# carlosmwh1985/BspAtom

Measured on AMD Instinct MI355X. Metric: l-channel eigensolves/sec at N_bsp=4096 fp64, higher is better.
Workload: dtype f64; 1 GPU; Hydrogen Coulomb l=0..127, N_bsp=4096, k=9, KIND_GRID=0 rb=800 (BASELINE configs[3]); `value` = weak scaling: 128 l-channels per GPU, 128 in total; channels_total=128, eigenvector_owner_rank=0, collective_calls=0, launched_by=python

## Files before the change

### bspatom_amd/csrc/common.h

```cpp
#pragma once
#include <hip/hip_runtime.h>
#include <cstdint>
#include <cstdio>
#include <cstdlib>

#define BSP_OK 0
#define BSP_ERR_HIP (-1)
#define BSP_ERR_ARG (-2)
#define BSP_ERR_BSPLVB (-3)
#define BSP_ERR_NOGPU (-4)
#define BSP_ERR_UNSUPPORTED (-5)

#define BSP_HIP(x)                                                                          \
    do {                                                                                    \
        hipError_t e_ = (x);                                                                \
        if (e_ != hipSuccess) {                                                             \
            fprintf(stderr, "bspatom: HIP error '%s' at %s:%d\n", hipGetErrorString(e_),    \
                    __FILE__, __LINE__);                                                    \
            return BSP_ERR_HIP;                                                             \
        }                                                                                   \
    } while (0)

typedef double double4_t __attribute__((ext_vector_type(4)));

// ... 90 lines not shown
                    int part, hipStream_t st);
int symm_lower_f64(int m, int batch, const double *A22, long ld, long bsA, const double *W, long ldw, long bsW,
                   double *Y, long ldy, long bsY, hipStream_t st);

int launch_point_table(int nkp, int k, int ka, int nfun, const double *d_rt, const double *d_aind,
                       const double *d_xg, const double *d_wg, const double *d_vpot, double *d_ptab,
                       int *d_left, int *d_status, hipStream_t st);
int launch_assemble_bands(int nfun, int k, int ka, int nkp, int kind_pot, const double *d_bl, int l0,
                          int nl, const double *d_ptab, const int *d_left, double *d_SB, double *d_HB,
                          hipStream_t st);
int launch_dipole_bands(int nfun, int k, int ka, int nkp, const double *d_ptab, const int *d_left, double *d_RB,
                        hipStream_t st);
int launch_band_cholesky(int n, int k, const double *d_SB, double *d_UB, double *d_rdiag, int *d_info,
                         hipStream_t st);
int launch_band_cholesky_range(int n, int k, int jstart, int jstop, const double *d_SB, double *d_UB, double *d_rdiag, int *d_info,
                               hipStream_t st);
int launch_band_cholesky_pair(int n, int k, int jstop, const double *d_SB, double *d_UB, double *d_rdiag, int *d_info, hipStream_t st);
int launch_standard_form(int n, int npad, int k, int nl, const double *d_HB, const double *d_UB,
                         const double *d_rdiag, double *d_Y, double *d_C, hipStream_t st, int full = 0);
struct CrawfordWork {
    double *SBf, *UBf, *rdiagf;
    double *Qel, *LiB;
    double *D, *E, *G;
    int *info;
};
bool crawford_supported(int n, int k);
size_t crawford_work_bytes(int n, int k, int nl);
void crawford_carve(void *base, int n, int k, int nl, CrawfordWork *w);
constexpr int CW_CHUNKS = 4;
int crawford_prepare(int n, int k, const double *d_SB, const CrawfordWork &w, hipStream_t st, hipEvent_t *evc = nullptr);
int crawford_run(int n, int npad, int k, int nl, const double *d_SB, const double *d_HB, const CrawfordWork &w, double *d_AB,
                 hipStream_t st, bool s_prepared = false, hipEvent_t *evc = nullptr, hipStream_t aux0 = nullptr);
long tsqr_scr_doubles(int npad);
long tsqr_cntr_ints(int npad);
int tsqr_panel(int npad, int r0, int c0, int batch, double *d_A, double *buf, double *W, double *scr, int *cntr, hipStream_t st);
struct Sy2sbWork {
    double *tsqr_scr;
    int *tsqr_cntr;
    double *buf2;
    double *tau2;
    double *buf;
    double *W;
    double *G;
    double *T;
    double *Kmat;
    double *tau;
// ... 127 lines not shown
```

### bspatom_amd/csrc/crawford.hip

```cpp
#include "common.h"
#include <cstdio>
#include <mutex>

namespace bsp {
namespace {

constexpr int CB = 8;
constexpr int CBB = CB * CB;

template <int CTRL>
__device__ __forceinline__ double cw_dpp(double x)
{
    union { double d; int i[2]; } u, r;
    u.d = x;
    r.i[0] = __builtin_amdgcn_update_dpp(0, u.i[0], CTRL, 0xf, 0xf, true);
    r.i[1] = __builtin_amdgcn_update_dpp(0, u.i[1], CTRL, 0xf, 0xf, true);
    return r.d;
}
__device__ __forceinline__ double cw_rowsum(double x)
{
    x += cw_dpp<0x128>(x);
    x += cw_dpp<0x124>(x);
    x += cw_dpp<0x122>(x);
    x += cw_dpp<0x121>(x);
    return x;
}
__device__ __forceinline__ double cw_bperm(double x, int srclane)
{
    union { double d; int i[2]; } u, r;
    u.d = x;
    r.i[0] = __builtin_amdgcn_ds_bpermute(srclane << 2, u.i[0]);
// ... 30 lines not shown
    if (I > 0) {
        const double w0 = cw_rowsum(x0 * u);
        x0 = fma(-t * w0, u, x0);
    }
    if (I > 4) {
        const double w1 = cw_rowsum(x1 * u);
        x1 = fma(-t * w1, u, x1);
    }
    if (g == GI) xr = (c < LEN) ? 0.0 : ((c == LEN) ? beta : xr);
#pragma unroll
    for (int r = 0; r < 4; ++r) {
        const double wq = cw_rowsum(q[r] * u);
        q[r] = fma(-t * wq, u, q[r]);
    }
}

__device__ __forceinline__ double4_t cw_mfma(double a, double b, double4_t acc)
{
    return __builtin_amdgcn_mfma_f64_16x16x4f64(a, b, acc, 0, 0, 0);
}

template <bool ONEDIV>
__global__ __launch_bounds__(256) void crawford_item_kernel(int N, int t, int jlo, int nch, int jel, int nlh, int qstride, int nlead,
                                                           const double *__restrict__ Qel, double *Dall, double *Eall, double *Gall)
{
    if ((int)blockIdx.y >= nlh) {
        if (jlo + nch > nlead) nch = nlead > jlo ? nlead - jlo : 0;
        if (jel >= nlead) jel = 0;
    }
    const int lane = threadIdx.x & 63;
    const int idx = blockIdx.x * 4 + __builtin_amdgcn_readfirstlane(threadIdx.x >> 6);
    const int g = lane >> 4, c = lane & 15, c8 = c & 7;
    const bool left = c < CB;
    bool elim;
    int j, p;
    if (idx < nch) { elim = false; j = jlo + idx; p = j - 2 - (t - 2 * j); }
    else if (idx == nch && jel > 0) { elim = true; j = jel; p = j - 1; }
    else return;
    const size_t chn = (size_t)blockIdx.y * N * CBB;
    double *D = Dall + chn, *E = Eall + chn, *G = Gall + chn;
    double *D0 = D + (size_t)p * CBB, *D1 = D0 + CBB, *E0 = E + (size_t)p * CBB;

    double w[4], sd[2];
#pragma unroll
    for (int r = 0; r < 2; ++r) {
        const int R = 4 * r + g;
        const int hi = R > c8 ? R : c8, lo = R > c8 ? c8 : R;
        w[r] = *(left ? D0 + hi * CB + lo : E0 + c8 * CB + R);
        w[r + 2] = *(left ? E0 + R * CB + c8 : D1 + hi * CB + lo);
    }
    const bool side = p >= 1;
    {
        const double *Em = E + (size_t)(side ? p - 1 : 0) * CBB;
#pragma unroll
        for (int r = 0; r < 2; ++r) {
            const double v = Em[(4 * r + g) * CB + c8];
            sd[r] = (side && left) ? v : 0.0;
        }
    }
    double q[4], x0 = 0.0, x1 = 0.0, xt[2] = {0.0, 0.0};
    const bool has_x = elim && (j + 1 <= N - 1);
    if (!elim) {
        const double *src = left ? G + (size_t)p * CBB + c8 : E + (size_t)(p + 1) * CBB + c8;
        x0 = src[g * CB];
        x1 = src[(4 + g) * CB];
#pragma unroll
        for (int r = 0; r < 4; ++r) q[r] = (4 * r + g == c) ? 1.0 : 0.0;
        rq_step<7, ONEDIV>(x0, x1, q, g, c);
        rq_step<6, ONEDIV>(x0, x1, q, g, c);
        rq_step<5, ONEDIV>(x0, x1, q, g, c);
        rq_step<4, ONEDIV>(x0, x1, q, g, c);
        rq_step<3, ONEDIV>(x0, x1, q, g, c);
// ... 4 lines not shown
        const double *Qj = Qel + ((int)blockIdx.y >= nlh ? qstride : 0) + (size_t)j * 256;
#pragma unroll
        for (int r = 0; r < 4; ++r) q[r] = Qj[(4 * r + g) * 16 + c];
        const double *Ej = E + (size_t)(has_x ? j : 0) * CBB;
#pragma unroll
        for (int r = 0; r < 2; ++r) {
            const double v = Ej[c8 * CB + 4 * r + g];
            xt[r] = (has_x && left) ? v : 0.0;
        }
    }

    double4_t P = {0.0, 0.0, 0.0, 0.0}, Wn = {0.0, 0.0, 0.0, 0.0};
#pragma unroll
    for (int r = 0; r < 4; ++r) P = cw_mfma(w[r], q[r], P);
#pragma unroll
    for (int r = 0; r < 4; ++r) Wn = cw_mfma(q[r], P[r], Wn);
    double4_t O = {0.0, 0.0, 0.0, 0.0};
    O = cw_mfma(q[0], sd[0], O);
    O = cw_mfma(q[1], sd[1], O);

    if (left) {
#pragma unroll
        for (int r = 0; r < 2; ++r) {
            D0[(4 * r + g) * CB + c8] = Wn[r];
            E0[(4 * r + g) * CB + c8] = Wn[r + 2];
        }
    } else {
#pragma unroll
        for (int r = 0; r < 2; ++r) D1[(4 * r + g) * CB + c8] = Wn[r + 2];
    }
    if (side && left) {
        double *Em = E + (size_t)(p - 1) * CBB, *Gm = G + (size_t)(p - 1) * CBB;
#pragma unroll
        for (int r = 0; r < 2; ++r) {
            if (!elim) Em[(4 * r + g) * CB + c8] = O[r];
            Gm[(4 * r + g) * CB + c8] = O[r + 2];
        }
    }
    if (!elim) {
        if (!left) {
            double *E1 = E + (size_t)(p + 1) * CBB;
            E1[g * CB + c8] = x0;
            E1[(4 + g) * CB + c8] = x1;
        }
    } else if (has_x) {
        double4_t T = {0.0, 0.0, 0.0, 0.0};
        T = cw_mfma(q[2], xt[0], T);
        T = cw_mfma(q[3], xt[1], T);
        if (left) {
            double *Ej = E + (size_t)j * CBB;
#pragma unroll
            for (int r = 0; r < 2; ++r) Ej[c8 * CB + 4 * r + g] = T[r + 2];
// ... 155 lines not shown
        cw_baxpy<I, 0, 8>(x, u, tw);
        cw_baxpy<I, 8, I + 1>(x, u, tw);
    }
    {
        double ws[4] = {0.0, 0.0, 0.0, 0.0};
        cw_bdot<I, 0, 8>(ws, u, q);
        cw_bdot<I, 8, I + 1>(ws, u, q);
        const double w = (ws[0] + ws[1]) + (ws[2] + ws[3]);
        const double tw = -t * w;
        cw_baxpy<I, 0, 8>(q, u, tw);
        if constexpr (ONEDIV) {
            cw_baxpy<I, 8, I + 1>(q, u, tw);
        } else {
            if constexpr (I > 0) cw_baxpy_last<I, 8, I>(q, u, tw, -t, w);
            else q[LEN] = fma(-t, w, q[LEN]);
        }
    }
}

template <bool ONEDIV, bool BCAST>
__device__ __forceinline__ void cw_quad(const int N, const int t, const int jlo, int nch, int jel, const int ipw, const int nlh,
                                        const int qstride, const int nlead, const int chan, const int idx0, const int lane,
                                        double *Qsw, double *Bcw, double *Wsw, const double *__restrict__ Qel, double *Dall, double *Eall,
                                        double *Gall, unsigned long long *diag)
{
    unsigned long long ts0 = 0, tsa = 0, tsb = 0, tsc = 0, tsd = 0, tse = 0;
    if (diag) ts0 = __builtin_amdgcn_s_memtime();
    if (chan >= nlh) {
        if (jlo + nch > nlead) nch = nlead > jlo ? nlead - jlo : 0;
        if (jel >= nlead) jel = 0;
    }
    const int items = nch + (jel > 0 ? 1 : 0);
    if (idx0 >= items) return;
    const size_t chn = (size_t)chan * N * CBB;
    double *D = Dall + chn, *E = Eall + chn, *G = Gall + chn;

#pragma unroll
    for (int s = 0; s < 4; ++s) {
        const int idx = idx0 + s;
        const int kd = s >= ipw ? 0 : (idx < nch ? 1 : ((idx == nch && jel > 0) ? 2 : 0));
        if (kd != 0) {
            const int jx = kd == 1 ? jlo + idx : jel, p = kd == 2 ? jel - 1 : jx - 2 - (t - 2 * jx);
            const double *srcD = D + (size_t)p * CBB + 2 * lane;
            const double *srcE = E + (size_t)((lane < 32 || p < 1) ? p : p - 1) * CBB + 2 * (lane & 31);
            const unsigned ldsD = (unsigned)(size_t)(__attribute__((address_space(3))) void *)(Wsw + s * 4 * CBB);
            asm volatile("s_mov_b32 m0, %2\n\ts_nop 0\n\tglobal_load_lds_dwordx4 %0, off\n\t"
                         "s_mov_b32 m0, %3\n\ts_nop 0\n\tglobal_load_lds_dwordx4 %1, off"
                         :: "v"(srcD), "v"(srcE), "s"(ldsD), "s"(ldsD + 2 * CBB * 8) : "memory", "m0");
        }
    }

    double wv[4][4], sdv[4][2];
    auto read_ws = [&]() {
        const int g = lane >> 4, c8 = lane & 7;
        const bool left = (lane & 15) < CB;
#pragma unroll
        for (int s = 0; s < 4; ++s) {
            const double *W0 = Wsw + s * 4 * CBB, *W1 = W0 + CBB, *WE = W0 + 2 * CBB, *WM = W0 + 3 * CBB;
#pragma unroll
            for (int r = 0; r < 2; ++r) {
                const int R = 4 * r + g;
                const int hi = R > c8 ? R : c8, lo = R > c8 ? c8 : R;
                wv[s][r] = *(left ? W0 + hi * CB + lo : WE + c8 * CB + R);
                wv[s][r + 2] = *(left ? WE + R * CB + c8 : W1 + hi * CB + lo);
                sdv[s][r] = WM[(4 * r + g) * CB + c8];
            }
        }
    };

    if (idx0 < nch) {
        const int it = lane >> 4, r = lane & 15;
        const int idx = idx0 + it;
        const bool live = idx < nch && it < ipw && r < CB;
        const int j = jlo + (idx < nch ? idx : 0), p = j - 2 - (t - 2 * j);
        double x[16], q[16];
        {
            const double *gp = G + (size_t)p * CBB + (r & 7) * CB, *ep = E + (size_t)(p + 1) * CBB + (r & 7) * CB;
#pragma unroll
            for (int c = 0; c < CB; c += 2) {
                const double2 a = *reinterpret_cast<const double2 *>(gp + c), b = *reinterpret_cast<const double2 *>(ep + c);
                x[c] = live ? a.x : 0.0; x[c + 1] = live ? a.y : 0.0;
                x[CB + c] = live ? b.x : 0.0; x[CB + c + 1] = live ? b.y : 0.0;
            }
        }
#pragma unroll
        for (int c = 0; c < 16; ++c) q[c] = (c == r) ? 1.0 : 0.0;
        if (diag) { asm volatile("s_waitcnt vmcnt(0)" ::: "memory"); tsa = __builtin_amdgcn_s_memtime(); }
        if constexpr (BCAST) {
// ... 21 lines not shown
            double *ep = E + (size_t)(p + 1) * CBB + r * CB;
#pragma unroll
            for (int c = 0; c < CB; c += 2) *reinterpret_cast<double2 *>(ep + c) = make_double2(x[CB + c], x[CB + c + 1]);
        }
        if constexpr (BCAST) {
            asm volatile("s_waitcnt vmcnt(4)" ::: "memory");
            read_ws();
            asm volatile("" ::: "memory");
        }
        double *qs = Qsw + it * (16 * QLD) + r * QLD;
#pragma unroll
        for (int c = 0; c < 16; c += 2) *reinterpret_cast<double2 *>(qs + c) = make_double2(q[c], q[c + 1]);
    } else if constexpr (BCAST) {
        asm volatile("s_waitcnt vmcnt(0)" ::: "memory");
        read_ws();
    }
    if constexpr (BCAST) asm volatile("s_waitcnt lgkmcnt(0)" ::: "memory");
    else if (idx0 < nch) asm volatile("s_waitcnt vmcnt(4) lgkmcnt(0)" ::: "memory");
    else asm volatile("s_waitcnt vmcnt(0) lgkmcnt(0)" ::: "memory");
    if (diag) tsc = __builtin_amdgcn_s_memtime();
    int idx0b = idx0;
    size_t chnb = chn;
    asm volatile("" : "+s"(idx0b), "+s"(chnb));
    D = Dall + chnb; E = Eall + chnb; G = Gall + chnb;

    const int g = lane >> 4, c = lane & 15, c8 = c & 7;
    const bool left = c < CB;
    int kind[4], jj[4], pp[4];
    double qe[4], xt[2] = {0.0, 0.0};
    if constexpr (!BCAST) read_ws();
#pragma unroll
    for (int s = 0; s < 4; ++s) {
        const int idx = idx0b + s;
        kind[s] = s >= ipw ? 0 : (idx < nch ? 1 : ((idx == nch && jel > 0) ? 2 : 0));
        jj[s] = kind[s] == 1 ? jlo + idx : (kind[s] == 2 ? jel : jlo + idx0b);
        pp[s] = kind[s] == 2 ? jel - 1 : jj[s] - 2 - (t - 2 * jj[s]);
        if (kind[s] == 0) { jj[s] = jj[0]; pp[s] = pp[0]; }
#pragma unroll
        for (int r = 0; r < 2; ++r) sdv[s][r] = (pp[s] >= 1 && left) ? sdv[s][r] : 0.0;
    }
    int se = -1;
#pragma unroll
    for (int s = 0; s < 4; ++s) if (kind[s] == 2) se = s;
    const bool has_x = se >= 0 && (jel + 1 <= N - 1);
    if (se >= 0) {
        const double *Qj = Qel + ((int)chan >= nlh ? qstride : 0) + (size_t)jel * 256;
#pragma unroll
        for (int r = 0; r < 4; ++r) qe[r] = Qj[(4 * r + g) * 16 + c];
        const double *Ej = E + (size_t)(has_x ? jel : 0) * CBB;
#pragma unroll
        for (int r = 0; r < 2; ++r) {
            const double v = Ej[c8 * CB + 4 * r + g];
            xt[r] = (has_x && left) ? v : 0.0;
        }
    }
    if (diag) { asm volatile("s_waitcnt vmcnt(0)" ::: "memory"); tsd = __builtin_amdgcn_s_memtime(); }
#pragma unroll
    for (int s = 0; s < 4; ++s) {
        if (kind[s] == 0) break;
        const bool elim = kind[s] == 2;
        const int p = pp[s];
        double *D0 = D + (size_t)p * CBB, *D1 = D0 + CBB, *E0 = E + (size_t)p * CBB;
        double q[4];
        if (!elim) {
            const double *qs = Qsw + s * (16 * QLD);
#pragma unroll
            for (int r = 0; r < 4; ++r) q[r] = qs[(4 * r + g) * QLD + c];
        } else {
#pragma unroll
            for (int r = 0; r < 4; ++r) q[r] = qe[r];
        }
        double4_t P = {0.0, 0.0, 0.0, 0.0}, Wn = {0.0, 0.0, 0.0, 0.0};
#pragma unroll
        for (int r = 0; r < 4; ++r) P = cw_mfma(wv[s][r], q[r], P);
#pragma unroll
        for (int r = 0; r < 4; ++r) Wn = cw_mfma(q[r], P[r], Wn);
        double4_t O = {0.0, 0.0, 0.0, 0.0};
        O = cw_mfma(q[0], sdv[s][0], O);
        O = cw_mfma(q[1], sdv[s][1], O);
        if (left) {
#pragma unroll
            for (int r = 0; r < 2; ++r) {
                D0[(4 * r + g) * CB + c8] = Wn[r];
                E0[(4 * r + g) * CB + c8] = Wn[r + 2];
            }
        } else {
#pragma unroll
            for (int r = 0; r < 2; ++r) D1[(4 * r + g) * CB + c8] = Wn[r + 2];
        }
        if (p >= 1 && left) {
            double *Em = E + (size_t)(p - 1) * CBB, *Gm = G + (size_t)(p - 1) * CBB;
#pragma unroll
            for (int r = 0; r < 2; ++r) {
                if (!elim) Em[(4 * r + g) * CB + c8] = O[r];
                Gm[(4 * r + g) * CB + c8] = O[r + 2];
            }
        }
        if (elim && has_x) {
            double4_t T = {0.0, 0.0, 0.0, 0.0};
            T = cw_mfma(q[2], xt[0], T);
            T = cw_mfma(q[3], xt[1], T);
            if (left) {
                double *Ej = E + (size_t)jel * CBB;
#pragma unroll
                for (int r = 0; r < 2; ++r) Ej[c8 * CB + 4 * r + g] = T[r + 2];
            }
        }
    }
    if (diag) {
        tse = __builtin_amdgcn_s_memtime();
        asm volatile("s_waitcnt vmcnt(0)" ::: "memory");
        const unsigned long long tsf = __builtin_amdgcn_s_memtime();
        if (lane == 0) {
            const bool a = tsa != 0;
            atomicAdd(diag + 0, a ? tsa - ts0 : 0ull);
            atomicAdd(diag + 1, a ? tsb - tsa : 0ull);
            atomicAdd(diag + 2, a ? tsc - tsb : tsc - ts0);
            atomicAdd(diag + 3, tsd - tsc);
            atomicAdd(diag + 4, tse - tsd);
            atomicAdd(diag + 5, tsf - tse);
            atomicAdd(diag + 6, tsf - ts0);
            atomicAdd(diag + 7, 1ull);
        }
    }
}

template <bool ONEDIV, int NW, bool BCAST>
__global__ __launch_bounds__(64 * NW, (BCAST ? 16 : 8) / NW) void crawford_item4_kernel(int N, int t, int jlo, int nch, int jel, int ipw, int nlh, int qstride,
                                                            int nlead, const double *__restrict__ Qel, double *Dall, double *Eall, double *Gall,
                                                            unsigned long long *diag)
{
    __builtin_amdgcn_s_setprio(3);
    if (diag && (((blockIdx.x & 7) | (blockIdx.y & 7)) != 0)) diag = nullptr;
    __shared__ __attribute__((aligned(16))) double Qs[NW][4][16 * QLD];
    __shared__ __attribute__((aligned(16))) double Bc[BCAST ? 1 : NW][BCAST ? 1 : 4][BCAST ? 2 : 16];
    __shared__ __attribute__((aligned(16))) double Wsep[BCAST ? 1 : NW][BCAST ? 1 : 4][BCAST ? 2 : 4 * CBB];
    static_assert(16 * QLD >= 4 * CBB, "a slot of Q holds a slot of phase B's operands");
    double *Wsw = BCAST ? &Qs[0][0][0] : &Wsep[0][0][0];
    const int lane = threadIdx.x & 63;
    const int wave = __builtin_amdgcn_readfirstlane(threadIdx.x >> 6);
    cw_quad<ONEDIV, BCAST>(N, t, jlo, nch, jel, ipw, nlh, qstride, nlead, (int)blockIdx.y, (blockIdx.x * NW + wave) * ipw, lane,
                           &Qs[wave][0][0], BCAST ? nullptr : &Bc[wave][0][0], Wsw + wave * (BCAST ? 4 * 16 * QLD : 4 * 4 * CBB), Qel, Dall,
                           Eall, Gall, diag);
}

__global__ void crawford_flip_kernel(int n, int k, const double *__restrict__ SB, double *__restrict__ SBf)
{
    const int idx = blockIdx.x * blockDim.x + threadIdx.x;
    if (idx >= n * k) return;
    const int d = idx / n, i = idx % n;
    SBf[idx] = (i + d < n) ? SB[(size_t)d * n + (n - 1 - i - d)] : 0.0;
    SBf[(size_t)n * k + idx] = SB[idx];
}

__global__ __launch_bounds__(64) void crawford_setup_kernel(int n, int k, int fstride, int jfirst, const double *__restrict__ UB0,
                                                           double *__restrict__ LiB0, double *__restrict__ Qel0)
{
    __shared__ double Ld[CB][CB + 1], M[CB][CB + 1], Li[CB][CB + 1];
    const int j = jfirst + blockIdx.x, t = threadIdx.x, r = t >> 3, c = t & 7, b = k - 1;
    const double *UBf = UB0 + (size_t)blockIdx.y * k * n;
    double *LiB = LiB0 + (size_t)blockIdx.y * fstride * CBB, *Qel = Qel0 + (size_t)blockIdx.y * fstride * 256;
    const int i = CB * j + r;
    {
        const int ic = CB * j + c, d = r - c;
        double v = 0.0;
        if (i >= n) v = (r == c) ? 1.0 : 0.0;
// ... 12 lines not shown
        for (int rr = 0; rr < CB; ++rr) {
            double s = (rr == t) ? 1.0 : 0.0;
#pragma unroll
            for (int kk = 0; kk < CB; ++kk)
                if (kk < rr && kk >= t) s -= Ld[rr][kk] * x[kk];
            x[rr] = (rr >= t) ? s / Ld[rr][rr] : 0.0;
        }
#pragma unroll
        for (int rr = 0; rr < CB; ++rr) Li[rr][t] = x[rr];
    }
    __syncthreads();
    double kv = 0.0;
#pragma unroll
    for (int kk = 0; kk < CB; ++kk) kv += Li[r][kk] * M[kk][c];
    LiB[(size_t)j * CBB + t] = Li[r][c];
    double *Q = Qel + (size_t)j * 256;
    Q[r * 16 + c] = (r == c) ? 1.0 : 0.0;
    Q[c * 16 + CB + r] = -kv;
    Q[(CB + r) * 16 + c] = 0.0;
    Q[(CB + c) * 16 + CB + r] = Li[r][c];
}

__global__ __launch_bounds__(64) void crawford_init_kernel(int n, int k, int N, int nlh, int listride, const double *__restrict__ HBall,
                                                          const double *__restrict__ LiB, double *Dall, double *Eall)
{
    __shared__ double Ds[CB][CB + 1], Es[CB][CB + 1], Ls[CB][CB + 1], Ts[CB][CB + 1];
    const int p = blockIdx.x, t = threadIdx.x, r = t >> 3, c = t & 7, b = k - 1;
    const bool fwd = (int)blockIdx.y >= nlh;
    const double *HB = HBall + (size_t)(fwd ? blockIdx.y - nlh : blockIdx.y) * k * n;
    auto Hf = [&](int i, int i2) -> double {
        const int hi = i > i2 ? i : i2, lo = i > i2 ? i2 : i, d = hi - lo;
        return (hi < n && d <= b) ? HB[(size_t)d * n + (fwd ? lo : n - 1 - hi)] : 0.0;
    };
    double dv = Hf(CB * p + r, CB * p + c), ev = Hf(CB * (p + 1) + r, CB * p + c);
    if (p == 0) {
        Ds[r][c] = dv; Es[r][c] = ev; Ls[r][c] = LiB[(fwd ? listride : 0) + t];
        __syncthreads();
        double s = 0.0, e2 = 0.0;
#pragma unroll
        for (int kk = 0; kk < CB; ++kk) { s += Ls[r][kk] * Ds[kk][c]; e2 += Es[r][kk] * Ls[c][kk]; }
        Ts[r][c] = s;
        __syncthreads();
        s = 0.0;
#pragma unroll
        for (int kk = 0; kk < CB; ++kk) s += Ts[r][kk] * Ls[c][kk];
        dv = s; ev = e2;
    }
    const size_t o = ((size_t)blockIdx.y * N + p) * CBB + t;
    Dall[o] = dv;
    Eall[o] = ev;
}

__global__ __launch_bounds__(64) void crawford_cut_setup_kernel(int n, int k, int N, int Nh, int Nl, const double *__restrict__ SBf,
                                                               const double *__restrict__ LiB, double *__restrict__ Qel, int *info)
{
    __shared__ double A[CB][CB + 1], Lf[CB][CB + 1], T[CB][CB + 1], Gm[CB][CB + 1], Li[CB][CB + 1];
    const int t = threadIdx.x, r = t >> 3, c = t & 7, b = k - 1;
    const double *L0 = LiB + (size_t)(Nh - 1) * CBB, *L1 = LiB + (size_t)N * CBB + (size_t)(Nl - 1) * CBB;
    {
        const int d = CB + r - c;
        A[r][c] = (d <= b) ? SBf[(size_t)d * n + CB * (Nh - 1) + c] : 0.0;
        Lf[r][c] = L1[(CB - 1 - r) * CB + (CB - 1 - c)];
        Li[r][c] = 0.0;
    }
    __syncthreads();
    double v = 0.0;
#pragma unroll
    for (int q = 0; q < CB; ++q) v += Lf[r][q] * A[q][c];
    T[r][c] = v;
    __syncthreads();
    v = 0.0;
#pragma unroll
    for (int q = 0; q < CB; ++q) v += T[r][q] * L0[c * CB + q];
// ... 28 lines not shown
            for (int kk = 0; kk < CB; ++kk)
                if (kk < rr && kk >= t) sacc -= A[rr][kk] * x[kk];
            x[rr] = (rr >= t) ? sacc / A[rr][rr] : 0.0;
        }
#pragma unroll
        for (int rr = 0; rr < CB; ++rr) Li[rr][t] = x[rr];
    }
    __syncthreads();
    double kv = 0.0;
#pragma unroll
    for (int kk = 0; kk < CB; ++kk) kv += Li[r][kk] * Gm[kk][c];
    double *Q = Qel + (size_t)Nh * 256;
    Q[r * 16 + c] = (r == c) ? 1.0 : 0.0;
    Q[c * 16 + CB + r] = -kv;
    Q[(CB + r) * 16 + c] = 0.0;
    Q[(CB + c) * 16 + CB + r] = Li[r][c];
}

__global__ __launch_bounds__(64) void crawford_cut_prep_kernel(int N, int Nh, int Nl, int nl, int Nfull, const double *__restrict__ LiB,
                                                              double *Dall, double *Eall)
{
    __shared__ double X[CB][CB + 1], Lf[CB][CB + 1];
    const int t = threadIdx.x, r = t >> 3, c = t & 7;
    const size_t c0 = (size_t)blockIdx.x * N * CBB, c1 = (size_t)(nl + blockIdx.x) * N * CBB;
    const double *L1 = LiB + (size_t)Nfull * CBB + (size_t)(Nl - 1) * CBB;
    X[r][c] = Eall[c0 + (size_t)(Nh - 1) * CBB + t];
    Lf[r][c] = L1[(CB - 1 - r) * CB + (CB - 1 - c)];
    __syncthreads();
    double v = 0.0;
#pragma unroll
    for (int q = 0; q < CB; ++q) v += Lf[r][q] * X[q][c];
    Eall[c0 + (size_t)(Nh - 1) * CBB + t] = v;
    Dall[c0 + (size_t)Nh * CBB + t] = Dall[c1 + (size_t)(Nl - 1) * CBB + (CB - 1 - r) * CB + (CB - 1 - c)];
    Eall[c0 + (size_t)Nh * CBB + t] = Eall[c1 + (size_t)(Nl - 2) * CBB + (CB - 1 - c) * CB + (CB - 1 - r)];
}

__device__ __forceinline__ double cw_rdl(double x, int l)
{
    union { double d; int i[2]; } u, r;
    u.d = x;
    r.i[0] = __builtin_amdgcn_readlane(u.i[0], l);
    r.i[1] = __builtin_amdgcn_readlane(u.i[1], l);
    return r.d;
}
__global__ __launch_bounds__(64) void crawford_corner_kernel(int N, double *__restrict__ Dall, double *__restrict__ Eall)
{
    const int lane = threadIdx.x, i = lane & 7;
    const bool isE = lane < 8, isD = lane >= 8 && lane < 16;
    double *rowp = (isE ? Eall : Dall) + (size_t)blockIdx.x * N * CBB + i * CB;
    double a[CB];
#pragma unroll
    for (int c = 0; c < CB; ++c) a[c] = (isE || isD) ? rowp[c] : 0.0;
#pragma unroll
    for (int r = CB - 1; r >= 1; --r) {
        double v[CB], nrm2 = 0.0;
#pragma unroll
        for (int c = 0; c < CB; ++c) v[c] = c <= r ? cw_rdl(a[c], r) : 0.0;
#pragma unroll
        for (int c = 0; c < r; ++c) nrm2 = fma(v[c], v[c], nrm2);
        if (nrm2 == 0.0) continue;
        const double alpha = v[r], beta = -copysign(sqrt(fma(alpha, alpha, nrm2)), alpha);
        const double tau = (beta - alpha) / beta, scale = 1.0 / (alpha - beta);
#pragma unroll
        for (int c = 0; c < r; ++c) v[c] *= scale;
        v[r] = 1.0;
        double sdot = 0.0;
#pragma unroll
        for (int c = 0; c <= r; ++c) sdot = fma(a[c], v[c], sdot);
        sdot *= tau;
#pragma unroll
        for (int c = 0; c <= r; ++c) a[c] = fma(-sdot, v[c], a[c]);
        if (isE && i == r) {
#pragma unroll
            for (int c = 0; c < r; ++c) a[c] = 0.0;
            a[r] = beta;
        }
        double vi = 0.0;
#pragma unroll
        for (int c = 0; c <= r; ++c) vi = (i == c) ? v[c] : vi;
#pragma unroll
        for (int c = 0; c < CB; ++c) {
            double y = 0.0;
#pragma unroll
            for (int q = 0; q <= r; ++q) y = fma(v[q], cw_rdl(a[c], CB + q), y);
            if (isD) a[c] = fma(-tau * vi, y, a[c]);
        }
    }
    if (isE || isD) {
#pragma unroll
        for (int c = 0; c < CB; ++c) rowp[c] = a[c];
    }
}

__global__ void crawford_band_kernel(int n, int npad, int N, int hw, int Nh, int Ntot, int nl, const double *__restrict__ Dall,
                                     const double *__restrict__ Eall, double *__restrict__ ABall)
{
    const int idx = blockIdx.x * blockDim.x + threadIdx.x;
    if (idx >= npad * 32) return;
    const int j = idx >> 5, d = idx & 31;
    const size_t ch = blockIdx.y;
    double v = 0.0;
    if (j + d < n && d <= hw) {
        const int ihi = n - 1 - j, ilo = ihi - d;
        const int P = ihi >> 3, Pc = ilo >> 3;
        const int rr = ihi & 7, cc = ilo & 7;
        if (Nh == 0) {
            const double *blk = (P == Pc ? Dall : Eall) + (ch * N + Pc) * CBB;
            v = (P - Pc <= 1) ? blk[rr * CB + cc] : 0.0;
        } else if (P - Pc <= 1) {
            const double *t0 = (P == Pc ? Dall : Eall) + ch * N * CBB, *t1 = (P == Pc ? Dall : Eall) + (nl + ch) * N * CBB;
            if (Pc <= Nh) v = t0[(size_t)Pc * CBB + rr * CB + cc];
            else if (P == Pc) v = t1[(size_t)(Ntot - 1 - P) * CBB + (CB - 1 - cc) * CB + (CB - 1 - rr)];
            else v = t1[(size_t)(Ntot - 2 - Pc) * CBB + (CB - 1 - cc) * CB + (CB - 1 - rr)];
        }
    }
    ABall[ch * ab_stride(npad) + (size_t)j * 128 + d] = v;
}

}

size_t crawford_work_bytes(int n, int k, int nl)
{
    const size_t N = (n + CB - 1) / CB;
    return ((size_t)4 * k * n + 2 * n + 2 * N * 256 + 2 * N * CBB + (size_t)3 * nl * 2 * (N + 2) * CBB) * sizeof(double) + 64;
}

void crawford_carve(void *base, int n, int k, int nl, CrawfordWork *w)
{
    const size_t N = (n + CB - 1) / CB;
    double *p = static_cast<double *>(base);
    w->SBf = p; p += (size_t)2 * k * n;
    w->UBf = p; p += (size_t)2 * k * n;
    w->rdiagf = p; p += 2 * n;
    w->Qel = p; p += 2 * N * 256;
    w->LiB = p; p += 2 * N * CBB;
    w->D = p; p += (size_t)nl * 2 * (N + 2) * CBB;
    w->E = p; p += (size_t)nl * 2 * (N + 2) * CBB;
    w->G = p; p += (size_t)nl * 2 * (N + 2) * CBB;
    w->info = reinterpret_cast<int *>(p);
}

bool crawford_supported(int n, int k) { return k >= 2 && k - 1 <= CB && n >= 2 * CB; }

namespace {
struct CwShape { int N, Nl, Nh, Nproc, Ns; bool split; };
CwShape cw_shape(int n)
{
    CwShape c;
    c.N = (n + CB - 1) / CB;
    c.Nl = (opts().cw_split > 0 && n % CB == 0) ? (int)((long)c.N * (opts().cw_split > 50 ? 50 : opts().cw_split) / 100) : 0;
    c.split = c.Nl >= 3 && c.N - c.Nl >= 4;
    if (!c.split) c.Nl = 0;
    c.Nh = c.split ? c.N - c.Nl : 0;
    c.Nproc = c.split ? c.Nh : c.N;
    c.Ns = c.split ? c.Nh + 2 : c.N;
    return c;
}
int cw_chunk_cols(int n) { return n < opts().cw_chunk_min ? n + 128 : ((n + CW_CHUNKS - 1) / CW_CHUNKS + 127) / 128 * 128; }
}
// ... 30 lines not shown
    return BSP_OK;
}

int crawford_run(int n, int npad, int k, int nl, const double *d_SB, const double *d_HB, const CrawfordWork &w, double *d_AB,
                 hipStream_t st, bool s_prepared, hipEvent_t *evc, hipStream_t aux0)
{
    if (!crawford_supported(n, k)) return BSP_ERR_UNSUPPORTED;
    const int N = (n + CB - 1) / CB;
    int Nl = (opts().cw_split > 0 && n % CB == 0) ? (int)((long)N * (opts().cw_split > 50 ? 50 : opts().cw_split) / 100) : 0;
    const bool split = Nl >= 3 && N - Nl >= 4;
    if (!split) Nl = 0;
    const int Nh = split ? N - Nl : 0;
    const int Nproc = split ? Nh : N;
    const int Ns = split ? Nh + 2 : N;
    const int ny = split ? 2 * nl : nl;
    const int nlead = split ? Nl : 0x7fffffff;
    int rc;
    KScope kt(KS_CRAWFORD, st);
    if (!s_prepared && (rc = crawford_prepare(n, k, d_SB, w, st))) return rc;
    if (!s_prepared) evc = nullptr;
    const int ccb = cw_chunk_cols(n) / CB;
    int waited = 0;
    if (evc) BSP_HIP(hipStreamWaitEvent(st, evc[0], 0));
    hipLaunchKernelGGL(crawford_init_kernel, dim3(Nproc, ny), dim3(64), 0, st, n, k, Ns, nl, N * CBB, d_HB, w.LiB, w.D, w.E);
    BSP_HIP(hipGetLastError());
    const int qstride = N * 256;
    unsigned long long *dg = nullptr;
    if (opts().cw_diag && opts().cw_items4) {
        BSP_HIP(hipMalloc(reinterpret_cast<void **>(&dg), 8 * sizeof(unsigned long long)));
        BSP_HIP(hipMemsetAsync(dg, 0, 8 * sizeof(unsigned long long), st));
    }
    auto wavefront = [&](int t, int jlo, int nch, int jel, int cy, int c0 = 0, hipStream_t ws = nullptr) {
        if (!ws) ws = st;
        double *gD = w.D + (size_t)c0 * Ns * CBB, *gE = w.E + (size_t)c0 * Ns * CBB, *gG = w.G + (size_t)c0 * Ns * CBB;
        const int items = nch + (jel ? 1 : 0);
        if (opts().cw_items4) {
            const int nw = opts().cw_nw == 4 ? 4 : 1;
            const int ipw = (opts().cw_ipw == 1 || opts().cw_ipw == 2) ? opts().cw_ipw : 4;
            const int waves = (items + ipw - 1) / ipw;
            const dim3 grid((waves + nw - 1) / nw, cy), block(64 * nw);
            const size_t pad = (size_t)opts().cw_ldspad * 1024;
#define CW_LAUNCH4(OD, NWV, BC, G, B, LDS)                                                                                           \
    hipLaunchKernelGGL((crawford_item4_kernel<OD, NWV, BC>), G, B, LDS, ws, Ns, t, jlo, nch, jel, ipw, nl, qstride, nlead, w.Qel, gD, gE, gG, dg)
            if (opts().cw_bcast) {
                if (opts().cw_onediv) CW_LAUNCH4(true, 1, true, dim3(waves, cy), dim3(64), 0);
                else if (nw == 4) CW_LAUNCH4(false, 4, true, grid, block, 0);
                else CW_LAUNCH4(false, 1, true, grid, block, pad);
            } else {
                if (opts().cw_onediv) CW_LAUNCH4(true, 1, false, dim3(waves, cy), dim3(64), 0);
                else if (nw == 4) CW_LAUNCH4(false, 4, false, grid, block, 0);
                else CW_LAUNCH4(false, 1, false, grid, block, pad);
            }
#undef CW_LAUNCH4
        } else {
            const dim3 grid((items + 3) / 4, cy);
            if (opts().cw_onediv) hipLaunchKernelGGL(crawford_item_kernel<true>, grid, dim3(256), 0, ws, Ns, t, jlo, nch, jel, nl, qstride, nlead, w.Qel, gD, gE, gG);
            else hipLaunchKernelGGL(crawford_item_kernel<false>, grid, dim3(256), 0, ws, Ns, t, jlo, nch, jel, nl, qstride, nlead, w.Qel, gD, gE, gG);
        }
    };
    const int tmax = (Nproc >= 3) ? 3 * Nproc - 5 : (Nproc == 2 ? 1 : 0);
    int ngrp = 1;
    if (!split && !dg && opts().cw_streams > 1) {
        ngrp = opts().cw_streams > 4 ? 4 : opts().cw_streams;
        while (ngrp > 1 && nl / ngrp < 16) --ngrp;
    }
    static hipStream_t s_aux[3] = {nullptr, nullptr, nullptr};
    hipStream_t aux[3];
    hipEvent_t evf = nullptr, evj[3] = {nullptr, nullptr, nullptr};
    if (ngrp > 1) {
        static std::mutex mx;
        std::lock_guard<std::mutex> lk(mx);
        for (int g = 0; g < ngrp - 1; ++g)
            if (!s_aux[g] && !(g == 0 && aux0)) BSP_HIP(hipStreamCreateWithFlags(&s_aux[g], hipStreamNonBlocking));
        for (int g = 0; g < 3; ++g) aux[g] = (g == 0 && aux0) ? aux0 : s_aux[g];
        BSP_HIP(hipEventCreateWithFlags(&evf, hipEventDisableTiming));
        BSP_HIP(hipEventRecord(evf, st));
        for (int g = 0; g < ngrp - 1; ++g) BSP_HIP(hipStreamWaitEvent(aux[g], evf, 0));
    }
    for (int t = 1; t <= tmax; ++t) {
        const int jel = ((t & 1) && (t + 1) / 2 <= Nproc - 1) ? (t + 1) / 2 : 0;
// ... 19 lines not shown
        }
        hipEventDestroy(evf);
        for (int g = 0; g < ngrp - 1; ++g) hipEventDestroy(evj[g]);
    }
    if (evc)
        for (; waited < CW_CHUNKS - 1; ++waited) BSP_HIP(hipStreamWaitEvent(st, evc[waited + 1], 0));
    if (split) {
        hipLaunchKernelGGL(crawford_cut_prep_kernel, dim3(nl), dim3(64), 0, st, Ns, Nh, Nl, nl, N, w.LiB, w.D, w.E);
        wavefront(2 * Nh - 1, 0, 0, Nh, nl);
        for (int sft = 0; sft <= Nh - 2; ++sft) wavefront(2 * Nh + sft, Nh, 1, 0, nl);
    }
    BSP_HIP(hipGetLastError());
    if (dg) {
        unsigned long long h[8];
        BSP_HIP(hipStreamSynchronize(st));
        BSP_HIP(hipMemcpy(h, dg, sizeof(h), hipMemcpyDeviceToHost));
        hipFree(dg);
        const double wv = h[7] ? (double)h[7] : 1.0;
        fprintf(stderr, "crawford_item4_kernel, %llu waves, s_memtime ticks per wave: X arrives %.0f | eight reflectors %.0f | R, Q stored %.0f | "
                        "phase B operands arrive %.0f | congruences issued %.0f | stores leave %.0f | wave %.0f\n", h[7], h[0] / wv, h[1] / wv,
                h[2] / wv, h[3] / wv, h[4] / wv, h[5] / wv, h[6] / wv);
    }
    const bool band8 = opts().cw_band8 != 0;
    if (band8) hipLaunchKernelGGL(crawford_corner_kernel, dim3(ny), dim3(64), 0, st, Ns, w.D, w.E);
    hipLaunchKernelGGL(crawford_band_kernel, dim3((npad * 32 + 255) / 256, nl), dim3(256), 0, st, n, npad, Ns, band8 ? CB : 2 * CB - 1,
                       Nh, N, nl, w.D, w.E, d_AB);
    BSP_HIP(hipGetLastError());
    return BSP_OK;
}

}
```

Measured before the change: 2093 eigensolves/s.

## Store Crawford diagonal blocks in packed lower-triangular form

The symmetric 8x8 diagonal blocks D are now stored as packed lower triangles (36 doubles instead of 64), with the strict upper triangle of block 0 kept in a small side array U for the corner kernel. Loads into LDS mask the exec to the packed size, and stores write only the lower triangle. This cuts global memory traffic and footprint for the D blocks across the wavefront, init, cut-prep, corner and band kernels. The cost is more index arithmetic and divergent masked stores, and the workspace carve places U inside the old D region.

```diff
diff --git a/bspatom_amd/csrc/common.h b/bspatom_amd/csrc/common.h
--- a/bspatom_amd/csrc/common.h
+++ b/bspatom_amd/csrc/common.h
@@ -136,6 +136,7 @@
     double *SBf, *UBf, *rdiagf;
     double *Qel, *LiB;
     double *D, *E, *G;
+    double *U;
     int *info;
 };
 bool crawford_supported(int n, int k);
diff --git a/bspatom_amd/csrc/crawford.hip b/bspatom_amd/csrc/crawford.hip
--- a/bspatom_amd/csrc/crawford.hip
+++ b/bspatom_amd/csrc/crawford.hip
@@ -7,6 +7,11 @@
 
 constexpr int CB = 8;
 constexpr int CBB = CB * CB;
+constexpr int CWD = CB * (CB + 1) / 2;
+constexpr int CWU = CBB - CWD;
+__host__ __device__ constexpr int cw_pk(int i, int j) { return i * (i + 1) / 2 + j; }
+__host__ __device__ constexpr int cw_up(int i, int j) { return cw_pk(j - 1, i); }
+static_assert(cw_pk(CB - 1, CB - 1) == CWD - 1 && cw_up(CB - 2, CB - 1) == CWU - 1, "the last places of the two triangles");
 
 template <int CTRL>
 __device__ __forceinline__ double cw_dpp(double x)
@@ -83,7 +88,7 @@
 
 template <bool ONEDIV>
 __global__ __launch_bounds__(256) void crawford_item_kernel(int N, int t, int jlo, int nch, int jel, int nlh, int qstride, int nlead,
-                                                           const double *__restrict__ Qel, double *Dall, double *Eall, double *Gall)
+                                                           const double *__restrict__ Qel, double *Dall, double *Eall, double *Gall, double *Uall)
 {
     if ((int)blockIdx.y >= nlh) {
         if (jlo + nch > nlead) nch = nlead > jlo ? nlead - jlo : 0;
@@ -99,16 +104,16 @@
     else if (idx == nch && jel > 0) { elim = true; j = jel; p = j - 1; }
     else return;
     const size_t chn = (size_t)blockIdx.y * N * CBB;
-    double *D = Dall + chn, *E = Eall + chn, *G = Gall + chn;
-    double *D0 = D + (size_t)p * CBB, *D1 = D0 + CBB, *E0 = E + (size_t)p * CBB;
+    double *D = Dall + (size_t)blockIdx.y * N * CWD, *E = Eall + chn, *G = Gall + chn, *U0 = Uall + (size_t)blockIdx.y * CWU;
+    double *D0 = D + (size_t)p * CWD, *D1 = D0 + CWD, *E0 = E + (size_t)p * CBB;
 
     double w[4], sd[2];
 #pragma unroll
     for (int r = 0; r < 2; ++r) {
         const int R = 4 * r + g;
         const int hi = R > c8 ? R : c8, lo = R > c8 ? c8 : R;
-        w[r] = *(left ? D0 + hi * CB + lo : E0 + c8 * CB + R);
-        w[r + 2] = *(left ? E0 + R * CB + c8 : D1 + hi * CB + lo);
+        w[r] = *(left ? D0 + cw_pk(hi, lo) : E0 + c8 * CB + R);
+        w[r + 2] = *(left ? E0 + R * CB + c8 : D1 + cw_pk(hi, lo));
     }
     const bool side = p >= 1;
     {
@@ -159,12 +164,17 @@
     if (left) {
 #pragma unroll
         for (int r = 0; r < 2; ++r) {
-            D0[(4 * r + g) * CB + c8] = Wn[r];
-            E0[(4 * r + g) * CB + c8] = Wn[r + 2];
+            const int R = 4 * r + g;
+            if (R >= c8) D0[cw_pk(R, c8)] = Wn[r];
+            else if (p == 0) U0[cw_up(R, c8)] = Wn[r];
+            E0[R * CB + c8] = Wn[r + 2];
         }
     } else {
 #pragma unroll
-        for (int r = 0; r < 2; ++r) D1[(4 * r + g) * CB + c8] = Wn[r + 2];
+        for (int r = 0; r < 2; ++r) {
+            const int R = 4 * r + g;
+            if (R >= c8) D1[cw_pk(R, c8)] = Wn[r + 2];
+        }
     }
     if (side && left) {
         double *Em = E + (size_t)(p - 1) * CBB, *Gm = G + (size_t)(p - 1) * CBB;
@@ -366,7 +376,7 @@
 __device__ __forceinline__ void cw_quad(const int N, const int t, const int jlo, int nch, int jel, const int ipw, const int nlh,
                                         const int qstride, const int nlead, const int chan, const int idx0, const int lane,
                                         double *Qsw, double *Bcw, double *Wsw, const double *__restrict__ Qel, double *Dall, double *Eall,
-                                        double *Gall, unsigned long long *diag)
+                                        double *Gall, double *Uall, unsigned long long *diag)
 {
     unsigned long long ts0 = 0, tsa = 0, tsb = 0, tsc = 0, tsd = 0, tse = 0;
     if (diag) ts0 = __builtin_amdgcn_s_memtime();
@@ -376,8 +386,8 @@
     }
     const int items = nch + (jel > 0 ? 1 : 0);
     if (idx0 >= items) return;
-    const size_t chn = (size_t)chan * N * CBB;
-    double *D = Dall + chn, *E = Eall + chn, *G = Gall + chn;
+    const size_t chn = (size_t)chan * N;
+    double *D = Dall + chn * CWD, *E = Eall + chn * CBB, *G = Gall + chn * CBB;
 
 #pragma unroll
     for (int s = 0; s < 4; ++s) {
@@ -385,12 +395,13 @@
         const int kd = s >= ipw ? 0 : (idx < nch ? 1 : ((idx == nch && jel > 0) ? 2 : 0));
         if (kd != 0) {
             const int jx = kd == 1 ? jlo + idx : jel, p = kd == 2 ? jel - 1 : jx - 2 - (t - 2 * jx);
-            const double *srcD = D + (size_t)p * CBB + 2 * lane;
+            const double *srcD = D + (size_t)p * CWD + 2 * lane;
             const double *srcE = E + (size_t)((lane < 32 || p < 1) ? p : p - 1) * CBB + 2 * (lane & 31);
             const unsigned ldsD = (unsigned)(size_t)(__attribute__((address_space(3))) void *)(Wsw + s * 4 * CBB);
-            asm volatile("s_mov_b32 m0, %2\n\ts_nop 0\n\tglobal_load_lds_dwordx4 %0, off\n\t"
-                         "s_mov_b32 m0, %3\n\ts_nop 0\n\tglobal_load_lds_dwordx4 %1, off"
-                         :: "v"(srcD), "v"(srcE), "s"(ldsD), "s"(ldsD + 2 * CBB * 8) : "memory", "m0");
+            unsigned long long ex;
+            asm volatile("s_mov_b32 m0, %3\n\ts_mov_b64 %0, exec\n\ts_bfm_b64 exec, %5, 0\n\tglobal_load_lds_dwordx4 %1, off\n\t"
+                         "s_mov_b64 exec, %0\n\ts_mov_b32 m0, %4\n\ts_nop 0\n\tglobal_load_lds_dwordx4 %2, off"
+                         : "=&s"(ex) : "v"(srcD), "v"(srcE), "s"(ldsD), "s"(ldsD + 2 * CBB * 8), "i"(CWD) : "memory", "m0");
         }
     }
 
@@ -398,16 +409,23 @@
     auto read_ws = [&]() {
         const int g = lane >> 4, c8 = lane & 7;
         const bool left = (lane & 15) < CB;
+        int oa[2], ob[2], om[2];
+#pragma unroll
+        for (int r = 0; r < 2; ++r) {
+            const int R = 4 * r + g;
+            const int hi = R > c8 ? R : c8, lo = R > c8 ? c8 : R;
+            oa[r] = left ? cw_pk(hi, lo) : 2 * CBB + c8 * CB + R;
+            ob[r] = left ? 2 * CBB + R * CB + c8 : CWD + cw_pk(hi, lo);
+            om[r] = 3 * CBB + R * CB + c8;
+        }
 #pragma unroll
         for (int s = 0; s < 4; ++s) {
-            const double *W0 = Wsw + s * 4 * CBB, *W1 = W0 + CBB, *WE = W0 + 2 * CBB, *WM = W0 + 3 * CBB;
+            const double *W0 = Wsw + s * 4 * CBB;
 #pragma unroll
             for (int r = 0; r < 2; ++r) {
-                const int R = 4 * r + g;
-                const int hi = R > c8 ? R : c8, lo = R > c8 ? c8 : R;
-                wv[s][r] = *(left ? W0 + hi * CB + lo : WE + c8 * CB + R);
-                wv[s][r + 2] = *(left ? WE + R * CB + c8 : W1 + hi * CB + lo);
-                sdv[s][r] = WM[(4 * r + g) * CB + c8];
+                wv[s][r] = W0[oa[r]];
+                wv[s][r + 2] = W0[ob[r]];
+                sdv[s][r] = W0[om[r]];
             }
         }
     };
@@ -475,11 +493,19 @@
     int idx0b = idx0;
     size_t chnb = chn;
     asm volatile("" : "+s"(idx0b), "+s"(chnb));
-    D = Dall + chnb; E = Eall + chnb; G = Gall + chnb;
+    D = Dall + chnb * CWD; E = Eall + chnb * CBB; G = Gall + chnb * CBB;
+    double *U0 = Uall + (size_t)chan * CWU;
 
     const int g = lane >> 4, c = lane & 15, c8 = c & 7;
     const bool left = c < CB;
     int kind[4], jj[4], pp[4];
+    int dk[2];
+    bool low[2];
+#pragma unroll
+    for (int r = 0; r < 2; ++r) {
+        low[r] = 4 * r + g >= c8;
+        dk[r] = (left ? 0 : CWD) + cw_pk(4 * r + g, c8);
+    }
     double qe[4], xt[2] = {0.0, 0.0};
     if constexpr (!BCAST) read_ws();
 #pragma unroll
@@ -513,7 +539,7 @@
         if (kind[s] == 0) break;
         const bool elim = kind[s] == 2;
         const int p = pp[s];
-        double *D0 = D + (size_t)p * CBB, *D1 = D0 + CBB, *E0 = E + (size_t)p * CBB;
+        double *D0 = D + (size_t)p * CWD, *E0 = E + (size_t)p * CBB;
         double q[4];
         if (!elim) {
             const double *qs = Qsw + s * (16 * QLD);
@@ -531,22 +557,26 @@
         double4_t O = {0.0, 0.0, 0.0, 0.0};
         O = cw_mfma(q[0], sdv[s][0], O);
         O = cw_mfma(q[1], sdv[s][1], O);
+        double wd[4] = {Wn[0], Wn[1], Wn[2], Wn[3]}, od[4] = {O[0], O[1], O[2], O[3]};
+        asm("" : "+v"(wd[0]), "+v"(wd[1]), "+v"(wd[2]), "+v"(wd[3]), "+v"(od[0]), "+v"(od[1]), "+v"(od[2]), "+v"(od[3]));
+#pragma unroll
+        for (int r = 0; r < 2; ++r)
+            if (low[r]) D0[dk[r]] = left ? wd[r] : wd[r + 2];
         if (left) {
 #pragma unroll
-            for (int r = 0; r < 2; ++r) {
-                D0[(4 * r + g) * CB + c8] = Wn[r];
-                E0[(4 * r + g) * CB + c8] = Wn[r + 2];
-            }
-        } else {
-#pragma unroll
-            for (int r = 0; r < 2; ++r) D1[(4 * r + g) * CB + c8] = Wn[r + 2];
+            for (int r = 0; r < 2; ++r) E0[(4 * r + g) * CB + c8] = wd[r + 2];
+        }
+        if (p == 0) {
+#pragma unroll
+            for (int r = 0; r < 2; ++r)
+                if (left && !low[r]) U0[cw_up(4 * r + g, c8)] = wd[r];
         }
         if (p >= 1 && left) {
             double *Em = E + (size_t)(p - 1) * CBB, *Gm = G + (size_t)(p - 1) * CBB;
 #pragma unroll
             for (int r = 0; r < 2; ++r) {
-                if (!elim) Em[(4 * r + g) * CB + c8] = O[r];
-                Gm[(4 * r + g) * CB + c8] = O[r + 2];
+                if (!elim) Em[(4 * r + g) * CB + c8] = od[r];
+                Gm[(4 * r + g) * CB + c8] = od[r + 2];
             }
         }
         if (elim && has_x) {
@@ -581,7 +611,7 @@
 template <bool ONEDIV, int NW, bool BCAST>
 __global__ __launch_bounds__(64 * NW, (BCAST ? 16 : 8) / NW) void crawford_item4_kernel(int N, int t, int jlo, int nch, int jel, int ipw, int nlh, int qstride,
                                                             int nlead, const double *__restrict__ Qel, double *Dall, double *Eall, double *Gall,
-                                                            unsigned long long *diag)
+                                                            double *Uall, unsigned long long *diag)
 {
     __builtin_amdgcn_s_setprio(3);
     if (diag && (((blockIdx.x & 7) | (blockIdx.y & 7)) != 0)) diag = nullptr;
@@ -594,7 +624,7 @@
     const int wave = __builtin_amdgcn_readfirstlane(threadIdx.x >> 6);
     cw_quad<ONEDIV, BCAST>(N, t, jlo, nch, jel, ipw, nlh, qstride, nlead, (int)blockIdx.y, (blockIdx.x * NW + wave) * ipw, lane,
                            &Qs[wave][0][0], BCAST ? nullptr : &Bc[wave][0][0], Wsw + wave * (BCAST ? 4 * 16 * QLD : 4 * 4 * CBB), Qel, Dall,
-                           Eall, Gall, diag);
+                           Eall, Gall, Uall, diag);
 }
 
 __global__ void crawford_flip_kernel(int n, int k, const double *__restrict__ SB, double *__restrict__ SBf)
@@ -653,7 +683,7 @@
 }
 
 __global__ __launch_bounds__(64) void crawford_init_kernel(int n, int k, int N, int nlh, int listride, const double *__restrict__ HBall,
-                                                          const double *__restrict__ LiB, double *Dall, double *Eall)
+                                                          const double *__restrict__ LiB, double *Dall, double *Eall, double *Uall)
 {
     __shared__ double Ds[CB][CB + 1], Es[CB][CB + 1], Ls[CB][CB + 1], Ts[CB][CB + 1];
     const int p = blockIdx.x, t = threadIdx.x, r = t >> 3, c = t & 7, b = k - 1;
@@ -677,9 +707,10 @@
         for (int kk = 0; kk < CB; ++kk) s += Ts[r][kk] * Ls[c][kk];
         dv = s; ev = e2;
     }
-    const size_t o = ((size_t)blockIdx.y * N + p) * CBB + t;
-    Dall[o] = dv;
-    Eall[o] = ev;
+    const size_t o = (size_t)blockIdx.y * N + p;
+    if (r >= c) Dall[o * CWD + cw_pk(r, c)] = dv;
+    else if (p == 0) Uall[(size_t)blockIdx.y * CWU + cw_up(r, c)] = dv;
+    Eall[o * CBB + t] = ev;
 }
 
 __global__ __launch_bounds__(64) void crawford_cut_setup_kernel(int n, int k, int N, int Nh, int Nl, const double *__restrict__ SBf,
@@ -754,7 +785,7 @@
 {
     __shared__ double X[CB][CB + 1], Lf[CB][CB + 1];
     const int t = threadIdx.x, r = t >> 3, c = t & 7;
-    const size_t c0 = (size_t)blockIdx.x * N * CBB, c1 = (size_t)(nl + blockIdx.x) * N * CBB;
+    const size_t b0 = (size_t)blockIdx.x * N, b1 = (size_t)(nl + blockIdx.x) * N, c0 = b0 * CBB, c1 = b1 * CBB;
     const double *L1 = LiB + (size_t)Nfull * CBB + (size_t)(Nl - 1) * CBB;
     X[r][c] = Eall[c0 + (size_t)(Nh - 1) * CBB + t];
     Lf[r][c] = L1[(CB - 1 - r) * CB + (CB - 1 - c)];
@@ -763,7 +794,7 @@
 #pragma unroll
     for (int q = 0; q < CB; ++q) v += Lf[r][q] * X[q][c];
     Eall[c0 + (size_t)(Nh - 1) * CBB + t] = v;
-    Dall[c0 + (size_t)Nh * CBB + t] = Dall[c1 + (size_t)(Nl - 1) * CBB + (CB - 1 - r) * CB + (CB - 1 - c)];
+    if (r >= c) Dall[(b0 + Nh) * CWD + cw_pk(r, c)] = Dall[(b1 + Nl - 1) * CWD + cw_pk(CB - 1 - c, CB - 1 - r)];
     Eall[c0 + (size_t)Nh * CBB + t] = Eall[c1 + (size_t)(Nl - 2) * CBB + (CB - 1 - c) * CB + (CB - 1 - r)];
 }
 
@@ -775,14 +806,16 @@
     r.i[1] = __builtin_amdgcn_readlane(u.i[1], l);
     return r.d;
 }
-__global__ __launch_bounds__(64) void crawford_corner_kernel(int N, double *__restrict__ Dall, double *__restrict__ Eall)
+__global__ __launch_bounds__(64) void crawford_corner_kernel(int N, double *__restrict__ Dall, double *__restrict__ Eall,
+                                                            const double *__restrict__ Uall)
 {
     const int lane = threadIdx.x, i = lane & 7;
     const bool isE = lane < 8, isD = lane >= 8 && lane < 16;
-    double *rowp = (isE ? Eall : Dall) + (size_t)blockIdx.x * N * CBB + i * CB;
+    double *rowE = Eall + (size_t)blockIdx.x * N * CBB + i * CB, *recD = Dall + (size_t)blockIdx.x * N * CWD;
+    const double *upD = Uall + (size_t)blockIdx.x * CWU;
     double a[CB];
 #pragma unroll
-    for (int c = 0; c < CB; ++c) a[c] = (isE || isD) ? rowp[c] : 0.0;
+    for (int c = 0; c < CB; ++c) a[c] = isE ? rowE[c] : (isD ? (c <= i ? recD[cw_pk(i, c)] : upD[cw_up(i, c)]) : 0.0);
 #pragma unroll
     for (int r = CB - 1; r >= 1; --r) {
         double v[CB], nrm2 = 0.0;
@@ -818,9 +851,10 @@
             if (isD) a[c] = fma(-tau * vi, y, a[c]);
         }
     }
-    if (isE || isD) {
-#pragma unroll
-        for (int c = 0; c < CB; ++c) rowp[c] = a[c];
+#pragma unroll
+    for (int c = 0; c < CB; ++c) {
+        if (isE) rowE[c] = a[c];
+        else if (isD && c <= i) recD[cw_pk(i, c)] = a[c];
     }
 }
 
@@ -837,13 +871,13 @@
         const int P = ihi >> 3, Pc = ilo >> 3;
         const int rr = ihi & 7, cc = ilo & 7;
         if (Nh == 0) {
-            const double *blk = (P == Pc ? Dall : Eall) + (ch * N + Pc) * CBB;
-            v = (P - Pc <= 1) ? blk[rr * CB + cc] : 0.0;
+            if (P == Pc) v = Dall[(ch * N + Pc) * CWD + cw_pk(rr, cc)];
+            else if (P - Pc == 1) v = Eall[(ch * N + Pc) * CBB + rr * CB + cc];
         } else if (P - Pc <= 1) {
-            const double *t0 = (P == Pc ? Dall : Eall) + ch * N * CBB, *t1 = (P == Pc ? Dall : Eall) + (nl + ch) * N * CBB;
-            if (Pc <= Nh) v = t0[(size_t)Pc * CBB + rr * CB + cc];
-            else if (P == Pc) v = t1[(size_t)(Ntot - 1 - P) * CBB + (CB - 1 - cc) * CB + (CB - 1 - rr)];
-            else v = t1[(size_t)(Ntot - 2 - Pc) * CBB + (CB - 1 - cc) * CB + (CB - 1 - rr)];
+            const size_t b0 = ch * N, b1 = (nl + ch) * N;
+            if (P == Pc) v = Pc <= Nh ? Dall[(b0 + Pc) * CWD + cw_pk(rr, cc)]
+                                      : Dall[(b1 + Ntot - 1 - P) * CWD + cw_pk(CB - 1 - cc, CB - 1 - rr)];
+            else v = Pc <= Nh ? Eall[(b0 + Pc) * CBB + rr * CB + cc] : Eall[(b1 + Ntot - 2 - Pc) * CBB + (CB - 1 - cc) * CB + (CB - 1 - rr)];
         }
     }
     ABall[ch * ab_stride(npad) + (size_t)j * 128 + d] = v;
@@ -867,6 +901,7 @@
     w->Qel = p; p += 2 * N * 256;
     w->LiB = p; p += 2 * N * CBB;
     w->D = p; p += (size_t)nl * 2 * (N + 2) * CBB;
+    w->U = w->D + (size_t)nl * 2 * (N + 2) * CWD;
     w->E = p; p += (size_t)nl * 2 * (N + 2) * CBB;
     w->G = p; p += (size_t)nl * 2 * (N + 2) * CBB;
     w->info = reinterpret_cast<int *>(p);
@@ -943,7 +978,7 @@
     const int ccb = cw_chunk_cols(n) / CB;
     int waited = 0;
     if (evc) BSP_HIP(hipStreamWaitEvent(st, evc[0], 0));
-    hipLaunchKernelGGL(crawford_init_kernel, dim3(Nproc, ny), dim3(64), 0, st, n, k, Ns, nl, N * CBB, d_HB, w.LiB, w.D, w.E);
+    hipLaunchKernelGGL(crawford_init_kernel, dim3(Nproc, ny), dim3(64), 0, st, n, k, Ns, nl, N * CBB, d_HB, w.LiB, w.D, w.E, w.U);
     BSP_HIP(hipGetLastError());
     const int qstride = N * 256;
     unsigned long long *dg = nullptr;
@@ -953,7 +988,8 @@
     }
     auto wavefront = [&](int t, int jlo, int nch, int jel, int cy, int c0 = 0, hipStream_t ws = nullptr) {
         if (!ws) ws = st;
-        double *gD = w.D + (size_t)c0 * Ns * CBB, *gE = w.E + (size_t)c0 * Ns * CBB, *gG = w.G + (size_t)c0 * Ns * CBB;
+        double *gD = w.D + (size_t)c0 * Ns * CWD, *gE = w.E + (size_t)c0 * Ns * CBB, *gG = w.G + (size_t)c0 * Ns * CBB;
+        double *gU = w.U + (size_t)c0 * CWU;
         const int items = nch + (jel ? 1 : 0);
         if (opts().cw_items4) {
             const int nw = opts().cw_nw == 4 ? 4 : 1;
@@ -962,7 +998,7 @@
             const dim3 grid((waves + nw - 1) / nw, cy), block(64 * nw);
             const size_t pad = (size_t)opts().cw_ldspad * 1024;
 #define CW_LAUNCH4(OD, NWV, BC, G, B, LDS)                                                                                           \
-    hipLaunchKernelGGL((crawford_item4_kernel<OD, NWV, BC>), G, B, LDS, ws, Ns, t, jlo, nch, jel, ipw, nl, qstride, nlead, w.Qel, gD, gE, gG, dg)
+    hipLaunchKernelGGL((crawford_item4_kernel<OD, NWV, BC>), G, B, LDS, ws, Ns, t, jlo, nch, jel, ipw, nl, qstride, nlead, w.Qel, gD, gE, gG, gU, dg)
             if (opts().cw_bcast) {
                 if (opts().cw_onediv) CW_LAUNCH4(true, 1, true, dim3(waves, cy), dim3(64), 0);
                 else if (nw == 4) CW_LAUNCH4(false, 4, true, grid, block, 0);
@@ -975,8 +1011,8 @@
 #undef CW_LAUNCH4
         } else {
             const dim3 grid((items + 3) / 4, cy);
-            if (opts().cw_onediv) hipLaunchKernelGGL(crawford_item_kernel<true>, grid, dim3(256), 0, ws, Ns, t, jlo, nch, jel, nl, qstride, nlead, w.Qel, gD, gE, gG);
-            else hipLaunchKernelGGL(crawford_item_kernel<false>, grid, dim3(256), 0, ws, Ns, t, jlo, nch, jel, nl, qstride, nlead, w.Qel, gD, gE, gG);
+            if (opts().cw_onediv) hipLaunchKernelGGL(crawford_item_kernel<true>, grid, dim3(256), 0, ws, Ns, t, jlo, nch, jel, nl, qstride, nlead, w.Qel, gD, gE, gG, gU);
+            else hipLaunchKernelGGL(crawford_item_kernel<false>, grid, dim3(256), 0, ws, Ns, t, jlo, nch, jel, nl, qstride, nlead, w.Qel, gD, gE, gG, gU);
         }
     };
     const int tmax = (Nproc >= 3) ? 3 * Nproc - 5 : (Nproc == 2 ? 1 : 0);
@@ -1042,7 +1078,7 @@
                 h[2] / wv, h[3] / wv, h[4] / wv, h[5] / wv, h[6] / wv);
     }
     const bool band8 = opts().cw_band8 != 0;
-    if (band8) hipLaunchKernelGGL(crawford_corner_kernel, dim3(ny), dim3(64), 0, st, Ns, w.D, w.E);
+    if (band8) hipLaunchKernelGGL(crawford_corner_kernel, dim3(ny), dim3(64), 0, st, Ns, w.D, w.E, w.U);
     hipLaunchKernelGGL(crawford_band_kernel, dim3((npad * 32 + 255) / 256, nl), dim3(256), 0, st, n, npad, Ns, band8 ? CB : 2 * CB - 1,
                        Nh, N, nl, w.D, w.E, d_AB);
     BSP_HIP(hipGetLastError());
```

New measurement: 2123 eigensolves/s, median of 6. 1.01x the previous value.
